# mic-rud/Learned-Compression-of-Point-Cloud-Geometry-and-Attributes

Measured on AMD Instinct MI355X. Metric: encode+decode Mpoints/sec, higher is better.
Workload: dtype f32

## Files before the change

### learned-compression-of-point-cloud-geometry-and-attributes_amd/csrc/common.h

```cpp
#pragma once
#include <hip/hip_runtime.h>
#include <stdint.h>

#include "../../include/pcc_hip.h"

namespace pcc {

void set_error(const char* fmt, ...);

#define PCC_CHECK_HIP(expr)                                                              \
    do {                                                                                 \
        hipError_t _e = (expr);                                                          \
        if (_e != hipSuccess) {                                                          \
            pcc::set_error("%s:%d: %s -> %s", __FILE__, __LINE__, #expr, hipGetErrorString(_e)); \
            return PCC_ERR_HIP;                                                          \
        }                                                                                \
    } while (0)

#define PCC_REQUIRE(cond, ...)                      \
    do {                                            \
        if (!(cond)) {                              \
            pcc::set_error(__VA_ARGS__);            \
            return PCC_ERR_ARG;                     \
        }                                           \
// ... 10 lines not shown
    return (unsigned)b;
}

constexpr uint64_t KEY_EMPTY = 0xFFFFFFFFFFFFFFFFull;
constexpr int KEY_FIELD_BITS = 18;
constexpr uint32_t KEY_FIELD_MASK = (1u << KEY_FIELD_BITS) - 1u;
constexpr int KEY_Y_SHIFT = KEY_FIELD_BITS, KEY_X_SHIFT = 2 * KEY_FIELD_BITS, KEY_B_SHIFT = 3 * KEY_FIELD_BITS;
constexpr int COORD_BIAS = 1 << (KEY_FIELD_BITS - 1);
constexpr int COORD_LIMIT = 130000;
constexpr int BATCH_LIMIT = 1022;
constexpr int64_t COUNT_ERR_RANGE = -2;

__host__ __device__ __forceinline__ bool coord_in_range(int b, int x, int y, int z) {
    return (unsigned)b <= (unsigned)BATCH_LIMIT && (unsigned)(x + COORD_LIMIT) <= 2u * COORD_LIMIT &&
           (unsigned)(y + COORD_LIMIT) <= 2u * COORD_LIMIT && (unsigned)(z + COORD_LIMIT) <= 2u * COORD_LIMIT;
}

__host__ __device__ __forceinline__ uint64_t pack_key(int b, int x, int y, int z) {
    return ((uint64_t)((uint32_t)b & 0x3FFu) << KEY_B_SHIFT) | ((uint64_t)((uint32_t)(x + COORD_BIAS) & KEY_FIELD_MASK) << KEY_X_SHIFT) |
           ((uint64_t)((uint32_t)(y + COORD_BIAS) & KEY_FIELD_MASK) << KEY_Y_SHIFT) | (uint64_t)((uint32_t)(z + COORD_BIAS) & KEY_FIELD_MASK);
}

__host__ __device__ __forceinline__ uint32_t key_z(uint64_t key) { return (uint32_t)key & KEY_FIELD_MASK; }
__host__ __device__ __forceinline__ uint32_t key_y(uint64_t key) { return (uint32_t)(key >> KEY_Y_SHIFT) & KEY_FIELD_MASK; }
__host__ __device__ __forceinline__ uint32_t key_x(uint64_t key) { return (uint32_t)(key >> KEY_X_SHIFT) & KEY_FIELD_MASK; }

__device__ __forceinline__ uint64_t hash_key(uint64_t k) {
    k ^= k >> 30; k *= 0xbf58476d1ce4e5b9ull;
    k ^= k >> 27; k *= 0x94d049bb133111ebull;
    k ^= k >> 31;
    return k;
}

__device__ __forceinline__ uint64_t table_slot0(uint64_t key, uint64_t mask, int shift) {
    const uint32_t z = key_z(key);
    const uint32_t lo = (uint32_t)(key >> (shift + 3)), hi = (uint32_t)(key >> 32);
    uint32_t h = lo * 0x9E3779B1u + hi * 0x85EBCA77u;
    h ^= h >> 15; h *= 0x2C1B3C6Du;
    h ^= h >> 12; h *= 0x297A2D39u;
    h ^= h >> 15;
    return (((uint64_t)h << 3) | (((z >> shift) + (h >> 29)) & 7u)) & mask;
}
constexpr uint64_t TABLE_PROBE_STEP = 8;

__host__ __device__ __forceinline__ int grid_shift_of(int tensor_stride) {
    int s = 0;
    if (tensor_stride > 0 && (tensor_stride & (tensor_stride - 1)) == 0)
        while ((1 << s) < tensor_stride) ++s;
    return s;
}

__device__ __forceinline__ int table_find(const uint64_t* __restrict__ keys, const int32_t* __restrict__ vals,
                                          uint64_t mask, int shift, uint64_t key) {
    const uint64_t slot0 = table_slot0(key, mask, shift);
    uint64_t slot = slot0;
    for (uint64_t probe = 0; probe <= mask; probe += TABLE_PROBE_STEP) {
        const uint64_t k = keys[slot];
        if (k == key) return vals[slot];
        if (k == KEY_EMPTY) return -1;
        slot = (slot + TABLE_PROBE_STEP) & mask;
    }
    for (uint64_t probe = 1; probe <= mask; ++probe) {
        slot = (slot0 + probe) & mask;
        const uint64_t k = keys[slot];
        if (k == key) return vals[slot];
        if (k == KEY_EMPTY) return -1;
    }
    return -1;
}

__device__ __forceinline__ uint64_t table_claim(uint64_t* keys, uint64_t mask, int shift, uint64_t key) {
    const uint64_t slot0 = table_slot0(key, mask, shift);
    uint64_t slot = slot0;
    for (uint64_t probe = 0; probe <= mask; probe += TABLE_PROBE_STEP) {
// ... 35 lines not shown
```

### learned-compression-of-point-cloud-geometry-and-attributes_amd/csrc/coords.hip

```cpp
#include <stdarg.h>
#include <stdio.h>
#include <stdlib.h>

#include "common.h"
#include "first_rows.h"
#include "sort.h"

namespace pcc {

static thread_local char g_err[512] = "";
void set_error(const char* fmt, ...) {
    va_list ap;
    va_start(ap, fmt);
    vsnprintf(g_err, sizeof(g_err), fmt, ap);
    va_end(ap);
}
const char* last_error() { return g_err; }

constexpr int SCAN_BLOCK = 256;
constexpr int SCAN_ITEMS = 4;
constexpr int SCAN_TILE = SCAN_BLOCK * SCAN_ITEMS;

__device__ __forceinline__ int wave_inclusive_scan(int v, int lane) {
#pragma unroll
// ... 271 lines not shown
    __shared__ int4 rows[64];
    __shared__ unsigned rm[64];
    __shared__ unsigned hits_s;
    const int64_t row0 = (int64_t)blockIdx.x * 64;
    if (threadIdx.x < 64) {
        const int64_t r = row0 + threadIdx.x;
        rows[threadIdx.x] = (r < n_out) ? reinterpret_cast<const int4*>(out_coords)[r] : make_int4(0, 0, 0, 0);
        rm[threadIdx.x] = 0u;
    }
    if (threadIdx.x == 0) hits_s = 0u;
    __syncthreads();
    unsigned myhits = 0u;
    const int total = 64 * K;
    for (int e = threadIdx.x; e < total; e += 256) {
        const int lr = e / K, k = e - lr * K;
        const int64_t r = row0 + lr;
        if (r >= n_out) break;
        int dx, dy, dz;
        kernel_offset(ks, k, dx, dy, dz);
        const int4 c = rows[lr];
        const int x = c.y + dx * step, y = c.z + dy * step, z = c.w + dz * step;
        int idx = -1;
        const bool on_grid = parent_pitch <= 0 || (((x % parent_pitch) | (y % parent_pitch) | (z % parent_pitch)) == 0);
        if (on_grid) idx = table_find(keys, vals, mask, shift, pack_key(c.x, x, y, z));
        nbr[r * K + k] = idx;
        if (idx >= 0) { atomicOr(&rm[lr], 1u << k); ++myhits; }
    }
    if (myhits) atomicAdd(&hits_s, myhits);
    __syncthreads();
    if (row_mask && threadIdx.x < 64 && row0 + threadIdx.x < n_out) row_mask[row0 + threadIdx.x] = rm[threadIdx.x];
    if (threadIdx.x == 0 && pair_count && !row_mask && hits_s) atomicAdd(pair_count, (unsigned long long)hits_s);
}

template <bool POW2>
__global__ __launch_bounds__(256) void kernel_map27_kernel(const int32_t* __restrict__ out_coords, int64_t n_out,
                                                           const uint64_t* __restrict__ keys,
                                                           const int32_t* __restrict__ vals, uint64_t mask, int shift,
                                                           int step, int parent_pitch, int32_t* __restrict__ nbr,
                                                           uint32_t* __restrict__ row_mask,
                                                           unsigned long long* __restrict__ pair_count) {
    __shared__ uint64_t rowkey[64];
    __shared__ uint64_t dkey[27];
    __shared__ unsigned rm[64];
    __shared__ unsigned hits_s;
    __shared__ unsigned short queue[64 * 27];
    __shared__ int queue_n;
    const int64_t row0 = (int64_t)blockIdx.x * 64;
    if (threadIdx.x < 64) {
        const int64_t r = row0 + threadIdx.x;
        const int4 c = (r < n_out) ? reinterpret_cast<const int4*>(out_coords)[r] : make_int4(0, 0, 0, 0);
        rowkey[threadIdx.x] = pack_key(c.x, c.y, c.z, c.w);
        rm[threadIdx.x] = 0u;
    }
    if (threadIdx.x == 255) queue_n = 0;
    if (threadIdx.x >= 64 && threadIdx.x < 64 + 27) {
        const int k = threadIdx.x - 64;
        const int64_t dx = (int64_t)(k % 3 - 1) * step, dy = (int64_t)((k / 3) % 3 - 1) * step, dz = (int64_t)(k / 9 - 1) * step;
        dkey[k] = (uint64_t)(dx * (1ll << KEY_X_SHIFT) + dy * (1ll << KEY_Y_SHIFT) + dz);
    }
    if (threadIdx.x == 0) hits_s = 0u;
    __syncthreads();
    const int nrows = (int)((n_out - row0 < 64) ? (n_out - row0) : 64);
    const int total = nrows * 27;
    unsigned myhits = 0u;
    auto off_grid_key = [&](uint64_t key) {
        if (POW2) {
            const uint32_t m = (uint32_t)(parent_pitch - 1);
            return ((((uint32_t)key | (uint32_t)(key >> KEY_Y_SHIFT) | (uint32_t)(key >> KEY_X_SHIFT)) & m) != 0u);
        }
        const int z = (int)key_z(key) - COORD_BIAS, y = (int)key_y(key) - COORD_BIAS, x = (int)key_x(key) - COORD_BIAS;
        return (x % parent_pitch) != 0 || (y % parent_pitch) != 0 || (z % parent_pitch) != 0;
    };
    constexpr int U = 7;
    {
        uint64_t key[U], got[U];
        uint32_t slot[U];
        int val[U];
        bool live[U];
        int lr = threadIdx.x / 27, k = threadIdx.x - lr * 27;
#pragma unroll
        for (int j = 0; j < U; ++j) {
            const int e = threadIdx.x + 256 * j;
            const bool valid = e < total;
            key[j] = rowkey[valid ? lr : 0] + dkey[k];
            live[j] = valid && (parent_pitch <= 0 || !off_grid_key(key[j]));
            slot[j] = (uint32_t)table_slot0(key[j], mask, shift);
            lr += 9;
            k += 13;
            if (k >= 27) { k -= 27; ++lr; }
        }
#pragma unroll
        for (int j = 0; j < U; ++j) {
            got[j] = live[j] ? keys[slot[j]] : KEY_EMPTY;
            val[j] = live[j] ? vals[slot[j]] : -1;
        }
        lr = threadIdx.x / 27;
        k = threadIdx.x - lr * 27;
#pragma unroll
        for (int j = 0; j < U; ++j) {
            const int e = threadIdx.x + 256 * j;
            const int lr_j = lr, k_j = k;
            lr += 9;
            k += 13;
            if (k >= 27) { k -= 27; ++lr; }
            if (e >= total) continue;
            int idx = -1;
            if (live[j] && got[j] != KEY_EMPTY) {
                if (got[j] == key[j]) idx = val[j];
                else {
                    queue[atomicAdd(&queue_n, 1)] = (unsigned short)e;
                    continue;
                }
            }
            nbr[row0 * 27 + e] = idx;
            if (idx >= 0) { atomicOr(&rm[lr_j], 1u << k_j); ++myhits; }
        }
    }
    __syncthreads();
    const int qn = queue_n;
    for (int qi = threadIdx.x; qi < qn; qi += 256) {
        const int e = queue[qi];
        const int lr = e / 27, k = e - lr * 27;
        const uint64_t key = rowkey[lr] + dkey[k];
        const uint64_t slot0 = table_slot0(key, mask, shift);
        uint64_t kk[4];
        int vv[4];
#pragma unroll
        for (int i = 0; i < 4; ++i) {
            const uint64_t sl = (slot0 + (uint64_t)(i + 1) * TABLE_PROBE_STEP) & mask;
            kk[i] = keys[sl];
            vv[i] = vals[sl];
        }
        int idx = -1;
        bool open = true;
        const int lane_slots = (int)((mask + TABLE_PROBE_STEP) / TABLE_PROBE_STEP);
#pragma unroll
        for (int i = 0; i < 4; ++i) {
            if (!open) break;
            if (i + 1 >= lane_slots) break;
            if (kk[i] == key) { idx = vv[i]; open = false; }
            else if (kk[i] == KEY_EMPTY) { idx = -1; open = false; }
        }
        if (open) idx = table_find(keys, vals, mask, shift, key);
        nbr[row0 * 27 + e] = idx;
        if (idx >= 0) { atomicOr(&rm[lr], 1u << k); ++myhits; }
    }
    if (myhits) atomicAdd(&hits_s, myhits);
    __syncthreads();
    if (row_mask && threadIdx.x < nrows) row_mask[row0 + threadIdx.x] = rm[threadIdx.x];
    if (threadIdx.x == 0 && pair_count && !row_mask && hits_s) atomicAdd(pair_count, (unsigned long long)hits_s);
}

__global__ __launch_bounds__(256) void pair_count_kernel(const uint32_t* __restrict__ row_mask, int64_t n,
                                                         unsigned long long* __restrict__ pair_count) {
    __shared__ unsigned long long ws[4];
    unsigned long long v = 0;
    for (int64_t i = (int64_t)blockIdx.x * 256 + threadIdx.x; i < n; i += (int64_t)gridDim.x * 256) v += __popc(row_mask[i]);
#pragma unroll
    for (int d = 32; d >= 1; d >>= 1) v += __shfl_xor(v, d, 64);
    if ((threadIdx.x & 63) == 0) ws[threadIdx.x >> 6] = v;
    __syncthreads();
    if (threadIdx.x == 0) {
        const unsigned long long t = ws[0] + ws[1] + ws[2] + ws[3];
        if (t) atomicAdd(pair_count, t);
    }
}

__global__ __launch_bounds__(256) void gather_rows_kernel(const float* __restrict__ src, int c,
                                                          const int32_t* __restrict__ idx, int64_t n,
                                                          float* __restrict__ out, int accumulate) {
    const int64_t total = n * c;
    for (int64_t e = (int64_t)blockIdx.x * blockDim.x + threadIdx.x; e < total; e += (int64_t)gridDim.x * blockDim.x) {
        const int64_t r = e / c;
        const int col = (int)(e - r * c);
        const int32_t s = idx[r];
        const float v = (s >= 0) ? src[(int64_t)s * c + col] : 0.0f;
        out[e] = accumulate ? out[e] + v : v;
    }
}

__global__ __launch_bounds__(256) void scatter_rows_kernel(const float* __restrict__ src, int c,
// ... 148 lines not shown
int pcc_children(const int32_t* coords, int64_t n, int32_t ts, int32_t ksize, uint64_t* keys, int32_t* vals,
                 int64_t cap, int32_t* scratch, int32_t* out_coords, int64_t* out_count, void* stream) {
    PCC_REQUIRE(ksize == 2 || ksize == 3, "pcc_children: kernel size must be 2 or 3");
    PCC_REQUIRE(ts >= 2 && (ts % 2) == 0, "pcc_children: tensor stride %d is not even", ts);
    const int K = ksize * ksize * ksize;
    GenChildren gen{coords, n, ksize, ts / 2, grid_shift_of(ts / 2)};
    return unique_coords(gen, n * K, keys, vals, cap, scratch, out_coords, out_count, as_stream(stream));
}

int32_t pcc_small_paths(int32_t mask) {
    const int before = pcc::small_paths_value();
    if (mask >= 0) pcc::g_small_paths = mask & 7;
    return before;
}

int pcc_kernel_map(const int32_t* out_coords, int64_t n_out, const uint64_t* in_keys, const int32_t* in_vals,
                   int64_t in_cap, int32_t ksize, int32_t step, int32_t sign, int32_t* nbr, uint32_t* row_mask,
                   int64_t* pair_count, void* stream) {
    PCC_REQUIRE(ksize >= 1 && ksize <= 3, "pcc_kernel_map: kernel size must be 1..3");
    PCC_REQUIRE(sign == 1 || sign == -1, "pcc_kernel_map: sign must be +1/-1");
    PCC_REQUIRE(in_cap > 0 && (in_cap & (in_cap - 1)) == 0, "pcc_kernel_map: bad capacity");
    if (pair_count) PCC_CHECK_HIP(hipMemsetAsync(pair_count, 0, sizeof(int64_t), as_stream(stream)));
    if (n_out <= 0) return PCC_OK;
    const int K = ksize * ksize * ksize;
    PCC_REQUIRE(step >= 1, "pcc_kernel_map: step must be >= 1");
    const int in_stride = sign > 0 ? step : 2 * step;
    const int pitch = sign > 0 ? 0 : 2 * step;
    const bool pow2 = pitch == 0 || (pitch & (pitch - 1)) == 0;
    unsigned long long* pc = reinterpret_cast<unsigned long long*>(pair_count);
    const uint64_t tmask = (uint64_t)(in_cap - 1);
    const int tshift = grid_shift_of(in_stride);
    const unsigned nb = blocks_for(n_out, 64);
    hipStream_t st = as_stream(stream);
    if (ksize == 3) {
        if (pow2) hipLaunchKernelGGL(kernel_map27_kernel<true>, dim3(nb), dim3(256), 0, st, out_coords, n_out, in_keys, in_vals, tmask, tshift,
                                     sign * step, pitch, nbr, row_mask, pc);
        else hipLaunchKernelGGL(kernel_map27_kernel<false>, dim3(nb), dim3(256), 0, st, out_coords, n_out, in_keys, in_vals, tmask, tshift,
                                sign * step, pitch, nbr, row_mask, pc);
    } else {
        hipLaunchKernelGGL(kernel_map_kernel, dim3(nb), dim3(256), 0, st, out_coords, n_out, in_keys, in_vals, tmask, tshift, ksize, K,
                           sign * step, pitch, nbr, row_mask, pc);
    }
    if (pair_count && row_mask)
        hipLaunchKernelGGL(pair_count_kernel, dim3(blocks_for(n_out, 256 * 16, 512)), dim3(256), 0, st, row_mask, n_out, pc);
    PCC_LAUNCH_CHECK();
    return PCC_OK;
}

int pcc_pair_count(const uint32_t* row_mask, int64_t n_out, int64_t* pair_count, void* stream) {
    PCC_REQUIRE(pair_count != nullptr, "pcc_pair_count: no output");
    hipStream_t st = as_stream(stream);
    PCC_CHECK_HIP(hipMemsetAsync(pair_count, 0, sizeof(int64_t), st));
    if (n_out <= 0) return PCC_OK;
    hipLaunchKernelGGL(pair_count_kernel, dim3(blocks_for(n_out, 256 * 16, 512)), dim3(256), 0, st, row_mask, n_out,
                       reinterpret_cast<unsigned long long*>(pair_count));
    PCC_LAUNCH_CHECK();
    return PCC_OK;
}

int pcc_gather_rows(const float* src, int32_t c, const int32_t* idx, int64_t n, float* out, int32_t accumulate,
                    void* stream) {
    if (n <= 0 || c <= 0) return PCC_OK;
    hipLaunchKernelGGL(gather_rows_kernel, dim3(blocks_for(n * c, 256, 65536)), dim3(256), 0, as_stream(stream), src, c,
                       idx, n, out, accumulate);
    PCC_LAUNCH_CHECK();
    return PCC_OK;
}

int pcc_scatter_rows(const float* src, int32_t c, const int32_t* idx, int64_t n, float* out, void* stream) {
    if (n <= 0 || c <= 0) return PCC_OK;
    hipLaunchKernelGGL(scatter_rows_kernel, dim3(blocks_for(n * c, 256, 65536)), dim3(256), 0, as_stream(stream), src,
// ... 50 lines not shown
```

### learned-compression-of-point-cloud-geometry-and-attributes_amd/csrc/select.hip

```cpp
#include <stdlib.h>

#include "common.h"
#include "sort_small.h"

namespace pcc {

constexpr int TK_STRIDE = 264;
constexpr int TK_LDS_BATCHES = 16;

__device__ __forceinline__ uint32_t float_key(float v) {
    if (v != v) return 0xFFFFFFFFu;
    if (v == 0.0f) v = 0.0f;
    const uint32_t u = __float_as_uint(v);
    return (u & 0x80000000u) ? ~u : (u | 0x80000000u);
}

struct Key96 { uint32_t w[3]; };

__device__ __forceinline__ Key96 make_key(float logit, int4 c) {
    const uint64_t lo = ~pack_key(c.x, c.y, c.z, c.w);
    Key96 k;
    k.w[0] = float_key(logit);
    k.w[1] = (uint32_t)(lo >> 32);
    k.w[2] = (uint32_t)lo;
// ... 224 lines not shown
        return true;
    });
    const int nb = st[2];
    for (int i = t; i < n; i += 1024) {
        const int4 c = reinterpret_cast<const int4*>(coords)[i];
        uint8_t m = 0;
        if (c.x == 0 && nb <= 12) m = cmp_prefix(make_key(logits[(int64_t)i * ld], c), st, nb) >= 0 ? 1 : 0;
        mask[i] = m;
    }
    for (int i = t; i < TK_STRIDE; i += 1024) state[i] = i < 8 ? st[i] : 0;
}

__global__ __launch_bounds__(256) void mask_bit_counts_kernel(const uint32_t* __restrict__ row_mask, int64_t n,
                                                              uint32_t* __restrict__ counts) {
    __shared__ unsigned c[27];
    if (threadIdx.x < 27) c[threadIdx.x] = 0u;
    __syncthreads();
    unsigned mine[27];
#pragma unroll
    for (int b = 0; b < 27; ++b) mine[b] = 0u;
    for (int64_t i0 = (int64_t)blockIdx.x * 256; i0 < n; i0 += (int64_t)gridDim.x * 256) {
        const int64_t i = i0 + threadIdx.x;
        const uint32_t m = (i < n) ? row_mask[i] : 0u;
#pragma unroll
        for (int b = 0; b < 27; ++b) mine[b] += (unsigned)__popcll(__ballot((m >> b) & 1u));
    }
    if ((threadIdx.x & 63) == 0) {
#pragma unroll
        for (int b = 0; b < 27; ++b)
            if (mine[b]) atomicAdd(&c[b], mine[b]);
    }
    __syncthreads();
    if (threadIdx.x < 27 && c[threadIdx.x]) atomicAdd(&counts[threadIdx.x], c[threadIdx.x]);
}

__device__ __forceinline__ void order_bit_positions(const uint32_t* __restrict__ counts, int* pos_s) {
    if (threadIdx.x < 27) {
        const uint32_t mine = counts[threadIdx.x];
        int rank = 0;
        for (int b = 0; b < 27; ++b) {
            const uint32_t o = counts[b];
            rank += (o < mine || (o == mine && b < (int)threadIdx.x)) ? 1 : 0;
        }
        pos_s[threadIdx.x] = 26 - rank;
    }
    __syncthreads();
}

__device__ __forceinline__ uint32_t order_key_of(uint32_t m, const int* pos_s) {
    uint32_t key = 0u;
#pragma unroll
    for (int b = 0; b < 27; ++b) key |= ((m >> b) & 1u) << pos_s[b];
    return 0x7FFFFFFu - key;
}

__global__ __launch_bounds__(256) void order_keys32_kernel(const uint32_t* __restrict__ row_mask, int64_t n,
                                                           const uint32_t* __restrict__ counts, uint32_t* __restrict__ keys) {
    __shared__ int pos_s[27];
    order_bit_positions(counts, pos_s);
    const int64_t i = (int64_t)blockIdx.x * 256 + threadIdx.x;
    if (i >= n) return;
    const uint32_t m = row_mask[i] & 0x7FFFFFFu;
    keys[i] = order_key_of(m, pos_s);
}

__global__ __launch_bounds__(256) void order_keys64_kernel(const uint32_t* __restrict__ row_mask,
                                                           const int32_t* __restrict__ coords, int64_t n,
                                                           int block_log2, int ts, const uint32_t* __restrict__ counts,
                                                           uint64_t* __restrict__ keys) {
    __shared__ int pos_s[27];
    order_bit_positions(counts, pos_s);
    const int64_t i = (int64_t)blockIdx.x * 256 + threadIdx.x;
    if (i >= n) return;
    uint64_t key = order_key_of(row_mask[i] & 0x7FFFFFFu, pos_s);
    const int4 c = reinterpret_cast<const int4*>(coords)[i];
    const uint64_t bx = (uint64_t)(((c.y / ts) + 512) >> block_log2) & 0x3FF;
    const uint64_t by = (uint64_t)(((c.z / ts) + 512) >> block_log2) & 0x3FF;
    const uint64_t bz = (uint64_t)(((c.w / ts) + 512) >> block_log2) & 0x3FF;
    key |= ((((uint64_t)(c.x & 0x3) << 30) | (bx << 20) | (by << 10) | bz) << 32);
    keys[i] = key;
}

__device__ __forceinline__ uint32_t tile_or_mask(uint32_t m) {
#pragma unroll
    for (int d = 1; d < 32; d <<= 1) m |= __shfl_xor(m, d, 64);
    return m;
// ... 203 lines not shown
    return PCC_OK;
}

int64_t pcc_order_scratch_bytes(int64_t n) { return pcc_sort_scratch_bytes(n); }

int pcc_order_rows_by_mask(const uint32_t* row_mask, const int32_t* coords, int64_t n, int32_t block_log2,
                           int32_t tensor_stride, int32_t* order, uint32_t* group_mask32, void* scratch, int64_t scratch_bytes,
                           void* stream) {
    if (n <= 0) return PCC_OK;
    PCC_REQUIRE(n < (1ll << 31), "pcc_order_rows_by_mask: too many rows");
    PCC_REQUIRE(block_log2 < 0 || coords != nullptr, "pcc_order_rows_by_mask: block ordering needs coordinates");
    PCC_REQUIRE(block_log2 <= 10, "pcc_order_rows_by_mask: block_log2 out of range");
    PCC_REQUIRE(tensor_stride >= 1, "pcc_order_rows_by_mask: bad tensor stride");
    PCC_REQUIRE(scratch_bytes >= pcc_sort_scratch_bytes(n), "pcc_order_rows_by_mask: scratch too small");
    hipStream_t st = as_stream(stream);
    const SortScratch s = carve_sort_scratch(scratch, n);
    if (small_path_enabled(0) && block_log2 < 0 && n <= RS_SMALL_N) {
        rs_small_dispatch(rs_small_rounds((int)n), [&](auto r) {
            hipLaunchKernelGGL(order_small_kernel<decltype(r)::value>, dim3(1), dim3(RS_SMALL_THREADS), 0, st, row_mask, (int)n,
                               static_cast<uint32_t*>(s.keys_a), static_cast<uint32_t*>(s.keys_b), s.vals_x, order);
        });
    } else {
        uint32_t* bit_counts = s.tail;
        PCC_CHECK_HIP(hipMemsetAsync(bit_counts, 0, 27 * sizeof(uint32_t), st));
        hipLaunchKernelGGL(mask_bit_counts_kernel, dim3(blocks_for(n, 256 * 16, 512)), dim3(256), 0, st, row_mask, n, bit_counts);
        const int begin = 0, end = block_log2 >= 0 ? 64 : 27;
        const int digit_bits = block_log2 >= 0 ? 8 : radix_sort_order_digit_bits(n);
        const bool in_b = radix_sort_result_in_b(begin, end, digit_bits);
        int32_t* va = in_b ? s.vals_x : order;
        int32_t* vb = in_b ? order : s.vals_x;
        int rc;
        if (block_log2 < 0) {
            uint32_t* ka = static_cast<uint32_t*>(s.keys_a);
            hipLaunchKernelGGL(order_keys32_kernel, dim3(blocks_for(n, 256)), dim3(256), 0, st, row_mask, n, bit_counts, ka);
            rc = radix_sort_pairs_u32(ka, static_cast<uint32_t*>(s.keys_b), va, vb, true, n, begin, end, s.counters, st, digit_bits);
        } else {
            uint64_t* ka = static_cast<uint64_t*>(s.keys_a);
            hipLaunchKernelGGL(order_keys64_kernel, dim3(blocks_for(n, 256)), dim3(256), 0, st, row_mask, coords, n, block_log2, tensor_stride,
                               bit_counts, ka);
            rc = radix_sort_pairs_u64(ka, static_cast<uint64_t*>(s.keys_b), va, vb, true, n, begin, end, s.counters, st);
        }
        if (rc) return rc;
    }
    hipLaunchKernelGGL(group_masks_kernel, dim3(blocks_for(n, 256)), dim3(256), 0, st, order, row_mask, n, group_mask32);
    PCC_LAUNCH_CHECK();
    return PCC_OK;
}

int64_t pcc_small_map_max(void) {
    static int off = -1;
    if (off < 0) { const char* e = getenv("PCC_SMALL_MAP"); off = (e && e[0] == '0') ? 1 : 0; }
    return off ? 0 : SMALL_MAP_MAX;
}

int pcc_small_kernel_map(const int32_t* out_coords, int64_t n_out, const uint64_t* in_keys, const int32_t* in_vals, int64_t in_cap,
                         int32_t ksize, int32_t step, int32_t sign, int32_t* nbr, uint32_t* row_mask, int32_t* order,
                         uint32_t* group_mask32, void* scratch, int64_t scratch_bytes, void* stream) {
    PCC_REQUIRE(ksize == 2 || ksize == 3, "pcc_small_kernel_map: kernel size must be 2 or 3");
    PCC_REQUIRE(sign == 1 || sign == -1, "pcc_small_kernel_map: sign must be +1/-1");
    PCC_REQUIRE(in_cap > 0 && (in_cap & (in_cap - 1)) == 0, "pcc_small_kernel_map: bad capacity");
    PCC_REQUIRE(step >= 1, "pcc_small_kernel_map: step must be >= 1");
    PCC_REQUIRE(n_out >= 0 && n_out <= SMALL_MAP_MAX, "pcc_small_kernel_map: %lld rows exceed %d", (long long)n_out, SMALL_MAP_MAX);
    PCC_REQUIRE(scratch_bytes >= pcc_sort_scratch_bytes(n_out), "pcc_small_kernel_map: scratch too small");
    if (n_out <= 0) return PCC_OK;
    const int in_stride = sign > 0 ? step : 2 * step;
    const int pitch = sign > 0 ? 0 : 2 * step;
    const SortScratch s = carve_sort_scratch(scratch, n_out);
    auto launch = [&](auto kernel) {
// ... 35 lines not shown
```

### learned-compression-of-point-cloud-geometry-and-attributes_amd/csrc/sort.h

```cpp
#pragma once
#include "common.h"

namespace pcc {

static inline int64_t align256(int64_t v) { return (v + 255) / 256 * 256; }

int64_t scan_block_sums_elems(int64_t m);
int scan_flags(const int32_t* flags, int64_t m, int32_t* pos, int32_t* block_sums, int64_t* total, int inclusive,
               hipStream_t st, const int32_t* err = nullptr);

int radix_sort_passes(int begin_bit, int end_bit, int digit_bits = 8);
static inline bool radix_sort_result_in_b(int begin_bit, int end_bit, int digit_bits = 8) { return radix_sort_passes(begin_bit, end_bit, digit_bits) & 1; }
int64_t radix_sort_counter_bytes(int64_t n);
int radix_sort_order_digit_bits(int64_t n);
int radix_sort_pairs_u32(uint32_t* keys_a, uint32_t* keys_b, int32_t* vals_a, int32_t* vals_b, bool vals_are_iota, int64_t n,
                         int begin_bit, int end_bit, void* counters, hipStream_t st, int digit_bits = 8);
int radix_sort_pairs_u64(uint64_t* keys_a, uint64_t* keys_b, int32_t* vals_a, int32_t* vals_b, bool vals_are_iota, int64_t n,
                         int begin_bit, int end_bit, void* counters, hipStream_t st);

}
```

### learned-compression-of-point-cloud-geometry-and-attributes_amd/csrc/sort.hip

```cpp
#include "sort_small.h"

namespace pcc {

constexpr int RS_MID_ITEMS = 8;
constexpr int RS_MID_MAX_UNITS = 64;
constexpr int RS_BIG_ITEMS = 16;

template <class K, int ROUNDS, int DB>
__global__ __launch_bounds__(RS_SMALL_THREADS) void radix_sort_small_kernel(K* ka, K* kb, int32_t* va, int32_t* vb, int iota, int n,
                                                                           int begin_bit, int end_bit, int passes) {
    radix_sort_small_body<K, ROUNDS, DB>(ka, kb, va, vb, iota, n, begin_bit, end_bit, passes);
}

template <class K, int ITEMS, int DB>
__global__ __launch_bounds__(256) void radix_count_kernel(const K* __restrict__ keys, int64_t n, int shift, unsigned dmask,
                                                          int64_t nunits, int32_t* __restrict__ counts) {
    constexpr int ND = 1 << DB;
    __shared__ int cnt[ND];
#pragma unroll
    for (int d = threadIdx.x; d < ND; d += 256) cnt[d] = 0;
    __syncthreads();
    const int64_t base = (int64_t)blockIdx.x * (256 * ITEMS);
    K key[ITEMS];
#pragma unroll
    for (int j = 0; j < ITEMS; ++j) {
        const int64_t i = base + (int64_t)j * 256 + threadIdx.x;
        key[j] = (i < n) ? keys[i] : (K)0;
    }
#pragma unroll
    for (int j = 0; j < ITEMS; ++j)
        if (base + (int64_t)j * 256 + threadIdx.x < n) atomicAdd(&cnt[(unsigned)(key[j] >> shift) & dmask], 1);
    __syncthreads();
#pragma unroll
    for (int d = threadIdx.x; d < ND; d += 256) counts[(int64_t)d * nunits + blockIdx.x] = cnt[d];
}

__global__ __launch_bounds__(256) void radix_rowscan_kernel(int32_t* __restrict__ counts, int64_t nunits, int32_t* __restrict__ totals) {
    __shared__ int wsum[4];
    __shared__ int carry_s;
    const int t = threadIdx.x, lane = t & 63, w = t >> 6;
    int32_t* row = counts + (int64_t)blockIdx.x * nunits;
    if (t == 0) carry_s = 0;
    __syncthreads();
    for (int64_t base = 0; base < nunits; base += 1024) {
        const int64_t i = base + 4 * (int64_t)t;
        int f[4];
        int v = 0;
#pragma unroll
        for (int j = 0; j < 4; ++j) {
            f[j] = (i + j < nunits) ? row[i + j] : 0;
            v += f[j];
        }
        const int inc = wave_inclusive_scan_i32(v, lane);
        if (lane == 63) wsum[w] = inc;
        __syncthreads();
        int pre = carry_s;
        for (int ww = 0; ww < w; ++ww) pre += wsum[ww];
        int ex = pre + inc - v;
#pragma unroll
        for (int j = 0; j < 4; ++j) {
            if (i + j < nunits) row[i + j] = ex;
            ex += f[j];
        }
        __syncthreads();
        if (t == 255) carry_s = pre + inc;
        __syncthreads();
    }
    if (t == 0) totals[blockIdx.x] = carry_s;
}

template <class K, int ITEMS, bool SELF_PREFIX, int DB>
__global__ __launch_bounds__(256) void radix_scatter_kernel(const K* __restrict__ src, K* __restrict__ dst, const int32_t* __restrict__ vs,
                                                            int32_t* __restrict__ vd, int iota, int64_t n, int shift, unsigned dmask,
                                                            int64_t nunits, const int32_t* __restrict__ counts,
                                                            const int32_t* __restrict__ totals) {
    constexpr int WAVE_KEYS = 64 * ITEMS, WG_KEYS = 4 * WAVE_KEYS;
    constexpr int ND = 1 << DB, DH = ND / 256;
    __shared__ K skey[WG_KEYS];
    __shared__ int32_t sval[WG_KEYS];
    __shared__ int cnt[4][ND];
    __shared__ int lbase[ND];
    __shared__ int gbase[ND];
    __shared__ int wsum[4], wsum2[4];
    const int t = threadIdx.x, lane = t & 63, w = t >> 6;
    const uint64_t lt = (1ull << lane) - 1ull;
    for (int i = t; i < 4 * ND; i += 256) (&cnt[0][0])[i] = 0;
    const int64_t base0 = (int64_t)blockIdx.x * WG_KEYS;
    const int64_t wbase = base0 + (int64_t)w * WAVE_KEYS;
    K key[ITEMS];
    int32_t val[ITEMS];
#pragma unroll
    for (int j = 0; j < ITEMS; ++j) {
        const int64_t i = wbase + j * 64 + lane;
        key[j] = (i < n) ? src[i] : (K)0;
        val[j] = (i < n) ? (iota ? (int32_t)i : vs[i]) : 0;
    }
    int pre[DH], total[DH];
#pragma unroll
    for (int h = 0; h < DH; ++h) {
        const int d = h * 256 + t;
        if (SELF_PREFIX) {
            const int32_t* row = counts + (int64_t)d * nunits;
            pre[h] = 0;
            total[h] = 0;
            for (int64_t u = 0; u < nunits; ++u) {
                const int c = row[u];
                total[h] += c;
                pre[h] += (u < (int64_t)blockIdx.x) ? c : 0;
            }
        } else {
            pre[h] = counts[(int64_t)d * nunits + blockIdx.x];
            total[h] = totals[d];
        }
    }
    __syncthreads();
#pragma unroll
    for (int j = 0; j < ITEMS; ++j)
        if (wbase + j * 64 + lane < n) atomicAdd(&cnt[w][(unsigned)(key[j] >> shift) & dmask], 1);
    __syncthreads();
    int gcarry = 0, lcarry = 0;
#pragma unroll
    for (int h = 0; h < DH; ++h) {
        const int d = h * 256 + t;
        const int c0 = cnt[0][d], c1 = cnt[1][d], c2 = cnt[2][d], c3 = cnt[3][d];
        const int mine = c0 + c1 + c2 + c3;
        const int inc = wave_inclusive_scan_i32(total[h], lane);
        const int linc = wave_inclusive_scan_i32(mine, lane);
// ... 25 lines not shown
        }
        __builtin_amdgcn_wave_barrier();
        if (active && below == 0) cnt[w][d] = base + __popcll(same);
        __builtin_amdgcn_wave_barrier();
    }
    __syncthreads();
    const int nk = (int)((n - base0 < WG_KEYS) ? (n - base0) : WG_KEYS);
    for (int i = t; i < nk; i += 256) {
        const K k = skey[i];
        const unsigned d = (unsigned)(k >> shift) & dmask;
        const int64_t pos = (int64_t)gbase[d] + (i - lbase[d]);
        dst[pos] = k;
        vd[pos] = sval[i];
    }
}

int radix_sort_passes(int begin_bit, int end_bit, int digit_bits) {
    return end_bit > begin_bit ? (end_bit - begin_bit + digit_bits - 1) / digit_bits : 0;
}

int radix_sort_order_digit_bits(int64_t n) {
    const int64_t mid_units = (n + 256 * RS_MID_ITEMS - 1) / (256 * RS_MID_ITEMS);
    return (n > RS_SMALL_N && mid_units <= RS_MID_MAX_UNITS) ? 8 : 9;
}

int64_t radix_sort_counter_bytes(int64_t n) {
    const int64_t mid = (n + 256 * RS_MID_ITEMS - 1) / (256 * RS_MID_ITEMS), big = (n + 256 * RS_BIG_ITEMS - 1) / (256 * RS_BIG_ITEMS);
    const int64_t nunits = mid <= RS_MID_MAX_UNITS ? mid : big;
    return align256(512 * (nunits > 0 ? nunits : 1) * 4) + 2048;
}

template <class K, int DB>
static int radix_sort_pairs(K* ka, K* kb, int32_t* va, int32_t* vb, bool iota, int64_t n, int begin_bit, int end_bit, void* counters,
                            hipStream_t st) {
    constexpr int ND = 1 << DB;
    const int passes = radix_sort_passes(begin_bit, end_bit, DB);
    PCC_REQUIRE(passes >= 1 && end_bit <= (int)(8 * sizeof(K)) && begin_bit >= 0, "radix sort: bad bit range [%d, %d)", begin_bit, end_bit);
    PCC_REQUIRE(n < (1ll << 31), "radix sort: too many keys (%lld)", (long long)n);
    if (n <= 0) return PCC_OK;
    if (n <= RS_SMALL_N) {
        rs_small_dispatch(rs_small_rounds((int)n), [&](auto r) {
            hipLaunchKernelGGL((radix_sort_small_kernel<K, decltype(r)::value, DB>), dim3(1), dim3(RS_SMALL_THREADS), 0, st, ka, kb, va, vb,
                               iota ? 1 : 0, (int)n, begin_bit, end_bit, passes);
        });
        PCC_LAUNCH_CHECK();
        return PCC_OK;
    }
    const int64_t mid_units = (n + 256 * RS_MID_ITEMS - 1) / (256 * RS_MID_ITEMS);
    const bool mid = mid_units <= RS_MID_MAX_UNITS;
    const int64_t nunits = mid ? mid_units : (n + 256 * RS_BIG_ITEMS - 1) / (256 * RS_BIG_ITEMS);
    int32_t* counts = reinterpret_cast<int32_t*>(counters);
    int32_t* totals = counts + align256((int64_t)ND * nunits * 4) / 4;
    K* src = ka;
    K* dst = kb;
    int32_t* vs = va;
    int32_t* vd = vb;
    for (int p = 0; p < passes; ++p) {
        const int shift = begin_bit + DB * p;
        const unsigned dmask = (end_bit - shift >= DB) ? (unsigned)(ND - 1) : ((1u << (end_bit - shift)) - 1u);
        const int io = (iota && p == 0) ? 1 : 0;
        if (mid) {
            hipLaunchKernelGGL((radix_count_kernel<K, RS_MID_ITEMS, DB>), dim3((unsigned)nunits), dim3(256), 0, st, src, n, shift, dmask, nunits, counts);
            hipLaunchKernelGGL((radix_scatter_kernel<K, RS_MID_ITEMS, true, DB>), dim3((unsigned)nunits), dim3(256), 0, st, src, dst, vs, vd, io, n,
                               shift, dmask, nunits, counts, totals);
        } else {
            hipLaunchKernelGGL((radix_count_kernel<K, RS_BIG_ITEMS, DB>), dim3((unsigned)nunits), dim3(256), 0, st, src, n, shift, dmask, nunits, counts);
            hipLaunchKernelGGL(radix_rowscan_kernel, dim3(ND), dim3(256), 0, st, counts, nunits, totals);
            hipLaunchKernelGGL((radix_scatter_kernel<K, RS_BIG_ITEMS, false, DB>), dim3((unsigned)nunits), dim3(256), 0, st, src, dst, vs, vd, io, n,
                               shift, dmask, nunits, counts, totals);
        }
        K* tk = src; src = dst; dst = tk;
        int32_t* tv = vs; vs = vd; vd = tv;
    }
    PCC_LAUNCH_CHECK();
    return PCC_OK;
}

int radix_sort_pairs_u32(uint32_t* keys_a, uint32_t* keys_b, int32_t* vals_a, int32_t* vals_b, bool vals_are_iota, int64_t n, int begin_bit,
                         int end_bit, void* counters, hipStream_t st, int digit_bits) {
    if (digit_bits == 9) return radix_sort_pairs<uint32_t, 9>(keys_a, keys_b, vals_a, vals_b, vals_are_iota, n, begin_bit, end_bit, counters, st);
    return radix_sort_pairs<uint32_t, 8>(keys_a, keys_b, vals_a, vals_b, vals_are_iota, n, begin_bit, end_bit, counters, st);
}

int radix_sort_pairs_u64(uint64_t* keys_a, uint64_t* keys_b, int32_t* vals_a, int32_t* vals_b, bool vals_are_iota, int64_t n, int begin_bit,
                         int end_bit, void* counters, hipStream_t st) {
    return radix_sort_pairs<uint64_t, 8>(keys_a, keys_b, vals_a, vals_b, vals_are_iota, n, begin_bit, end_bit, counters, st);
}

}
```

Baseline: 8.949.

## Share hashes across z-neighbours in map27 and fuse order-key build into radix sort

The 27-neighbour map kernel now has each thread handle three z-adjacent offsets. It reuses the run hash when those keys fall in the same hash run, reorders rows so run-crossing rows are grouped, and stages results in shared memory for vectorised int4 stores. The block size drops to 192 threads. Separately, for large sorts, the order-key generation kernel is fused into the first radix pass: keys are computed from the row masks through a per-block 3x512 lookup table instead of being written to memory first. This removes one kernel and one key round trip, but adds LUT setup to every count and scatter block.

```diff
diff --git a/learned-compression-of-point-cloud-geometry-and-attributes_amd/csrc/common.h b/learned-compression-of-point-cloud-geometry-and-attributes_amd/csrc/common.h
--- a/learned-compression-of-point-cloud-geometry-and-attributes_amd/csrc/common.h
+++ b/learned-compression-of-point-cloud-geometry-and-attributes_amd/csrc/common.h
@@ -66,14 +66,23 @@
     return k;
 }
 
-__device__ __forceinline__ uint64_t table_slot0(uint64_t key, uint64_t mask, int shift) {
-    const uint32_t z = key_z(key);
-    const uint32_t lo = (uint32_t)(key >> (shift + 3)), hi = (uint32_t)(key >> 32);
+__device__ __forceinline__ uint32_t table_run_lo(uint64_t key, int shift) { return (uint32_t)(key >> (shift + 3)); }
+__device__ __forceinline__ uint32_t table_run_hi(uint64_t key) { return (uint32_t)(key >> 32); }
+
+__device__ __forceinline__ uint32_t table_run_hash(uint32_t lo, uint32_t hi) {
     uint32_t h = lo * 0x9E3779B1u + hi * 0x85EBCA77u;
     h ^= h >> 15; h *= 0x2C1B3C6Du;
     h ^= h >> 12; h *= 0x297A2D39u;
     h ^= h >> 15;
+    return h;
+}
+
+__device__ __forceinline__ uint64_t table_run_slot(uint32_t h, uint32_t z, uint64_t mask, int shift) {
     return (((uint64_t)h << 3) | (((z >> shift) + (h >> 29)) & 7u)) & mask;
+}
+
+__device__ __forceinline__ uint64_t table_slot0(uint64_t key, uint64_t mask, int shift) {
+    return table_run_slot(table_run_hash(table_run_lo(key, shift), table_run_hi(key)), key_z(key), mask, shift);
 }
 constexpr uint64_t TABLE_PROBE_STEP = 8;
 
diff --git a/learned-compression-of-point-cloud-geometry-and-attributes_amd/csrc/coords.hip b/learned-compression-of-point-cloud-geometry-and-attributes_amd/csrc/coords.hip
--- a/learned-compression-of-point-cloud-geometry-and-attributes_amd/csrc/coords.hip
+++ b/learned-compression-of-point-cloud-geometry-and-attributes_amd/csrc/coords.hip
@@ -327,8 +327,9 @@
     if (threadIdx.x == 0 && pair_count && !row_mask && hits_s) atomicAdd(pair_count, (unsigned long long)hits_s);
 }
 
+constexpr int MAP27_ROWS = 64, MAP27_THREADS = 192, MAP27_COLS = 3;
 template <bool POW2>
-__global__ __launch_bounds__(256) void kernel_map27_kernel(const int32_t* __restrict__ out_coords, int64_t n_out,
+__global__ __launch_bounds__(MAP27_THREADS) void kernel_map27_kernel(const int32_t* __restrict__ out_coords, int64_t n_out,
                                                            const uint64_t* __restrict__ keys,
                                                            const int32_t* __restrict__ vals, uint64_t mask, int shift,
                                                            int step, int parent_pitch, int32_t* __restrict__ nbr,
@@ -340,14 +341,25 @@
     __shared__ unsigned hits_s;
     __shared__ unsigned short queue[64 * 27];
     __shared__ int queue_n;
+    __shared__ __attribute__((aligned(16))) int32_t stage[MAP27_ROWS * 27];
+    static_assert(MAP27_ROWS == 64 && MAP27_ROWS * 9 == MAP27_THREADS * MAP27_COLS && MAP27_THREADS >= 64 + 27, "lane mapping");
+    __shared__ unsigned char rowat[64];
     const int64_t row0 = (int64_t)blockIdx.x * 64;
+    const int nrows = (int)((n_out - row0 < 64) ? (n_out - row0) : 64);
     if (threadIdx.x < 64) {
         const int64_t r = row0 + threadIdx.x;
-        const int4 c = (r < n_out) ? reinterpret_cast<const int4*>(out_coords)[r] : make_int4(0, 0, 0, 0);
-        rowkey[threadIdx.x] = pack_key(c.x, c.y, c.z, c.w);
+        const bool valid = r < n_out;
+        const int4 c = valid ? reinterpret_cast<const int4*>(out_coords)[r] : make_int4(0, 0, 0, 0);
+        const uint64_t key = pack_key(c.x, c.y, c.z, c.w), dzkey = (uint64_t)(int64_t)step;
+        rowkey[threadIdx.x] = key;
         rm[threadIdx.x] = 0u;
-    }
-    if (threadIdx.x == 255) queue_n = 0;
+        const uint32_t lo = table_run_lo(key, shift);
+        const bool crosses = valid && (table_run_lo(key - dzkey, shift) != lo || table_run_lo(key + dzkey, shift) != lo);
+        const uint64_t cb = __ballot(crosses), sb = __ballot(valid && !crosses), below = (1ull << threadIdx.x) - 1ull;
+        const int at = !valid ? (int)threadIdx.x : crosses ? __popcll(cb & below) : __popcll(cb) + __popcll(sb & below);
+        rowat[at] = (unsigned char)threadIdx.x;
+    }
+    if (threadIdx.x == MAP27_THREADS - 1) queue_n = 0;
     if (threadIdx.x >= 64 && threadIdx.x < 64 + 27) {
         const int k = threadIdx.x - 64;
         const int64_t dx = (int64_t)(k % 3 - 1) * step, dy = (int64_t)((k / 3) % 3 - 1) * step, dz = (int64_t)(k / 9 - 1) * step;
@@ -355,7 +367,6 @@
     }
     if (threadIdx.x == 0) hits_s = 0u;
     __syncthreads();
-    const int nrows = (int)((n_out - row0 < 64) ? (n_out - row0) : 64);
     const int total = nrows * 27;
     unsigned myhits = 0u;
     auto off_grid_key = [&](uint64_t key) {
@@ -366,54 +377,78 @@
         const int z = (int)key_z(key) - COORD_BIAS, y = (int)key_y(key) - COORD_BIAS, x = (int)key_x(key) - COORD_BIAS;
         return (x % parent_pitch) != 0 || (y % parent_pitch) != 0 || (z % parent_pitch) != 0;
     };
-    constexpr int U = 7;
     {
-        uint64_t key[U], got[U];
-        uint32_t slot[U];
-        int val[U];
-        bool live[U];
-        int lr = threadIdx.x / 27, k = threadIdx.x - lr * 27;
+        constexpr int U = MAP27_COLS;
+        uint64_t key[U][3], got[U][3];
+        uint32_t slot[U][3];
+        int val[U][3];
+        bool live[U][3];
+        const uint64_t dzkey = (uint64_t)(int64_t)step;
+        const int ncols = nrows * 9;
+        int p = threadIdx.x / 9, c9 = threadIdx.x - p * 9;
+        int lr[U];
 #pragma unroll
         for (int j = 0; j < U; ++j) {
-            const int e = threadIdx.x + 256 * j;
-            const bool valid = e < total;
-            key[j] = rowkey[valid ? lr : 0] + dkey[k];
-            live[j] = valid && (parent_pitch <= 0 || !off_grid_key(key[j]));
-            slot[j] = (uint32_t)table_slot0(key[j], mask, shift);
-            lr += 9;
-            k += 13;
-            if (k >= 27) { k -= 27; ++lr; }
+            const bool valid = threadIdx.x + MAP27_THREADS * j < ncols;
+            lr[j] = valid ? rowat[p] : 0;
+            const uint64_t centre = rowkey[lr[j]] + dkey[9 + c9];
+            key[j][0] = centre - dzkey;
+            key[j][1] = centre;
+            key[j][2] = centre + dzkey;
+            uint32_t lo[3];
+#pragma unroll
+            for (int d = 0; d < 3; ++d) {
+                live[j][d] = valid && (parent_pitch <= 0 || !off_grid_key(key[j][d]));
+                lo[d] = table_run_lo(key[j][d], shift);
+            }
+            const uint32_t hi = table_run_hi(centre);
+            const uint32_t first = live[j][1] ? lo[1] : (live[j][0] ? lo[0] : lo[2]);
+#pragma unroll
+            for (int d = 0; d < 3; ++d) lo[d] = live[j][d] ? lo[d] : first;
+            const bool other0 = lo[0] != lo[1], other2 = lo[2] != lo[1];
+            const uint32_t h_a = table_run_hash(lo[1], hi);
+            uint32_t h_b = h_a;
+            if (other0 || other2) h_b = table_run_hash(other0 ? lo[0] : lo[2], hi);
+            uint32_t h_c = h_b;
+            if (other0 && other2 && lo[2] != lo[0]) h_c = table_run_hash(lo[2], hi);
+            const uint32_t h[3] = {other0 ? h_b : h_a, h_a, other2 ? (other0 ? h_c : h_b) : h_a};
+#pragma unroll
+            for (int d = 0; d < 3; ++d) slot[j][d] = (uint32_t)table_run_slot(h[d], key_z(key[j][d]), mask, shift);
+            p += 21;
+            c9 += 3;
+            if (c9 >= 9) { c9 -= 9; ++p; }
         }
 #pragma unroll
         for (int j = 0; j < U; ++j) {
-            got[j] = live[j] ? keys[slot[j]] : KEY_EMPTY;
-            val[j] = live[j] ? vals[slot[j]] : -1;
-        }
-        lr = threadIdx.x / 27;
-        k = threadIdx.x - lr * 27;
+#pragma unroll
+            for (int d = 0; d < 3; ++d) {
+                got[j][d] = live[j][d] ? keys[slot[j][d]] : KEY_EMPTY;
+                val[j][d] = live[j][d] ? vals[slot[j][d]] : -1;
+            }
+        }
+        c9 = threadIdx.x % 9;
 #pragma unroll
         for (int j = 0; j < U; ++j) {
-            const int e = threadIdx.x + 256 * j;
-            const int lr_j = lr, k_j = k;
-            lr += 9;
-            k += 13;
-            if (k >= 27) { k -= 27; ++lr; }
-            if (e >= total) continue;
-            int idx = -1;
-            if (live[j] && got[j] != KEY_EMPTY) {
-                if (got[j] == key[j]) idx = val[j];
-                else {
-                    queue[atomicAdd(&queue_n, 1)] = (unsigned short)e;
-                    continue;
-                }
+            const int lr_j = lr[j], c_j = c9;
+            c9 += 3;
+            if (c9 >= 9) c9 -= 9;
+            if (threadIdx.x + MAP27_THREADS * j >= ncols) continue;
+            unsigned bits = 0u;
+#pragma unroll
+            for (int d = 0; d < 3; ++d) {
+                const int k = c_j + 9 * d, e = 27 * lr_j + k;
+                const int idx = got[j][d] == key[j][d] ? val[j][d] : -1;
+                stage[e] = idx;
+                bits |= (idx >= 0 ? 1u : 0u) << k;
+                if (got[j][d] != key[j][d] && got[j][d] != KEY_EMPTY) queue[atomicAdd(&queue_n, 1)] = (unsigned short)e;
             }
-            nbr[row0 * 27 + e] = idx;
-            if (idx >= 0) { atomicOr(&rm[lr_j], 1u << k_j); ++myhits; }
+            myhits += __popc(bits);
+            if (bits) atomicOr(&rm[lr_j], bits);
         }
     }
     __syncthreads();
     const int qn = queue_n;
-    for (int qi = threadIdx.x; qi < qn; qi += 256) {
+    for (int qi = threadIdx.x; qi < qn; qi += MAP27_THREADS) {
         const int e = queue[qi];
         const int lr = e / 27, k = e - lr * 27;
         const uint64_t key = rowkey[lr] + dkey[k];
@@ -437,11 +472,15 @@
             else if (kk[i] == KEY_EMPTY) { idx = -1; open = false; }
         }
         if (open) idx = table_find(keys, vals, mask, shift, key);
-        nbr[row0 * 27 + e] = idx;
+        stage[e] = idx;
         if (idx >= 0) { atomicOr(&rm[lr], 1u << k); ++myhits; }
     }
     if (myhits) atomicAdd(&hits_s, myhits);
     __syncthreads();
+    int32_t* out = nbr + row0 * 27;
+    const int nvec = ((reinterpret_cast<uintptr_t>(out) & 15u) == 0u) ? total >> 2 : 0;
+    for (int i = threadIdx.x; i < nvec; i += MAP27_THREADS) reinterpret_cast<int4*>(out)[i] = reinterpret_cast<const int4*>(stage)[i];
+    for (int i = 4 * nvec + threadIdx.x; i < total; i += MAP27_THREADS) out[i] = stage[i];
     if (row_mask && threadIdx.x < nrows) row_mask[row0 + threadIdx.x] = rm[threadIdx.x];
     if (threadIdx.x == 0 && pair_count && !row_mask && hits_s) atomicAdd(pair_count, (unsigned long long)hits_s);
 }
@@ -656,11 +695,12 @@
     const int tshift = grid_shift_of(in_stride);
     const unsigned nb = blocks_for(n_out, 64);
     hipStream_t st = as_stream(stream);
+    static_assert(MAP27_ROWS == 64, "nb counts 64 rows per workgroup for every map kernel");
     if (ksize == 3) {
-        if (pow2) hipLaunchKernelGGL(kernel_map27_kernel<true>, dim3(nb), dim3(256), 0, st, out_coords, n_out, in_keys, in_vals, tmask, tshift,
-                                     sign * step, pitch, nbr, row_mask, pc);
-        else hipLaunchKernelGGL(kernel_map27_kernel<false>, dim3(nb), dim3(256), 0, st, out_coords, n_out, in_keys, in_vals, tmask, tshift,
-                                sign * step, pitch, nbr, row_mask, pc);
+        if (pow2) hipLaunchKernelGGL(kernel_map27_kernel<true>, dim3(nb), dim3(MAP27_THREADS), 0, st, out_coords, n_out, in_keys, in_vals, tmask,
+                                     tshift, sign * step, pitch, nbr, row_mask, pc);
+        else hipLaunchKernelGGL(kernel_map27_kernel<false>, dim3(nb), dim3(MAP27_THREADS), 0, st, out_coords, n_out, in_keys, in_vals, tmask,
+                                tshift, sign * step, pitch, nbr, row_mask, pc);
     } else {
         hipLaunchKernelGGL(kernel_map_kernel, dim3(nb), dim3(256), 0, st, out_coords, n_out, in_keys, in_vals, tmask, tshift, ksize, K,
                            sign * step, pitch, nbr, row_mask, pc);
diff --git a/learned-compression-of-point-cloud-geometry-and-attributes_amd/csrc/select.hip b/learned-compression-of-point-cloud-geometry-and-attributes_amd/csrc/select.hip
--- a/learned-compression-of-point-cloud-geometry-and-attributes_amd/csrc/select.hip
+++ b/learned-compression-of-point-cloud-geometry-and-attributes_amd/csrc/select.hip
@@ -280,26 +280,6 @@
     }
     __syncthreads();
     if (threadIdx.x < 27 && c[threadIdx.x]) atomicAdd(&counts[threadIdx.x], c[threadIdx.x]);
-}
-
-__device__ __forceinline__ void order_bit_positions(const uint32_t* __restrict__ counts, int* pos_s) {
-    if (threadIdx.x < 27) {
-        const uint32_t mine = counts[threadIdx.x];
-        int rank = 0;
-        for (int b = 0; b < 27; ++b) {
-            const uint32_t o = counts[b];
-            rank += (o < mine || (o == mine && b < (int)threadIdx.x)) ? 1 : 0;
-        }
-        pos_s[threadIdx.x] = 26 - rank;
-    }
-    __syncthreads();
-}
-
-__device__ __forceinline__ uint32_t order_key_of(uint32_t m, const int* pos_s) {
-    uint32_t key = 0u;
-#pragma unroll
-    for (int b = 0; b < 27; ++b) key |= ((m >> b) & 1u) << pos_s[b];
-    return 0x7FFFFFFu - key;
 }
 
 __global__ __launch_bounds__(256) void order_keys32_kernel(const uint32_t* __restrict__ row_mask, int64_t n,
@@ -569,8 +549,12 @@
         int rc;
         if (block_log2 < 0) {
             uint32_t* ka = static_cast<uint32_t*>(s.keys_a);
-            hipLaunchKernelGGL(order_keys32_kernel, dim3(blocks_for(n, 256)), dim3(256), 0, st, row_mask, n, bit_counts, ka);
-            rc = radix_sort_pairs_u32(ka, static_cast<uint32_t*>(s.keys_b), va, vb, true, n, begin, end, s.counters, st, digit_bits);
+            if (n > RS_SMALL_N) {
+                rc = radix_sort_order_u32(row_mask, bit_counts, ka, static_cast<uint32_t*>(s.keys_b), va, vb, n, s.counters, st, digit_bits);
+            } else {
+                hipLaunchKernelGGL(order_keys32_kernel, dim3(blocks_for(n, 256)), dim3(256), 0, st, row_mask, n, bit_counts, ka);
+                rc = radix_sort_pairs_u32(ka, static_cast<uint32_t*>(s.keys_b), va, vb, true, n, begin, end, s.counters, st, digit_bits);
+            }
         } else {
             uint64_t* ka = static_cast<uint64_t*>(s.keys_a);
             hipLaunchKernelGGL(order_keys64_kernel, dim3(blocks_for(n, 256)), dim3(256), 0, st, row_mask, coords, n, block_log2, tensor_stride,
diff --git a/learned-compression-of-point-cloud-geometry-and-attributes_amd/csrc/sort.h b/learned-compression-of-point-cloud-geometry-and-attributes_amd/csrc/sort.h
--- a/learned-compression-of-point-cloud-geometry-and-attributes_amd/csrc/sort.h
+++ b/learned-compression-of-point-cloud-geometry-and-attributes_amd/csrc/sort.h
@@ -18,4 +18,45 @@
 int radix_sort_pairs_u64(uint64_t* keys_a, uint64_t* keys_b, int32_t* vals_a, int32_t* vals_b, bool vals_are_iota, int64_t n,
                          int begin_bit, int end_bit, void* counters, hipStream_t st);
 
+__device__ __forceinline__ void order_bit_positions(const uint32_t* __restrict__ counts, int* pos_s) {
+    if (threadIdx.x < 27) {
+        const uint32_t mine = counts[threadIdx.x];
+        int rank = 0;
+        for (int b = 0; b < 27; ++b) {
+            const uint32_t o = counts[b];
+            rank += (o < mine || (o == mine && b < (int)threadIdx.x)) ? 1 : 0;
+        }
+        pos_s[threadIdx.x] = 26 - rank;
+    }
+    __syncthreads();
 }
+
+__device__ __forceinline__ uint32_t order_key_of(uint32_t m, const int* pos_s) {
+    uint32_t key = 0u;
+#pragma unroll
+    for (int b = 0; b < 27; ++b) key |= ((m >> b) & 1u) << pos_s[b];
+    return 0x7FFFFFFu - key;
+}
+
+constexpr int ORDER_LUT_SIZE = 3 * 512;
+__device__ __forceinline__ void order_key_tables(const uint32_t* __restrict__ counts, int* pos_s, uint32_t* lut) {
+    order_bit_positions(counts, pos_s);
+    for (int i = threadIdx.x; i < ORDER_LUT_SIZE; i += blockDim.x) {
+        const int third = i >> 9;
+        const uint32_t v = (uint32_t)i & 511u;
+        uint32_t image = 0u;
+#pragma unroll
+        for (int b = 0; b < 9; ++b) image |= ((v >> b) & 1u) << pos_s[9 * third + b];
+        lut[i] = image;
+    }
+    __syncthreads();
+}
+
+__device__ __forceinline__ uint32_t order_key_from_tables(uint32_t m, const uint32_t* lut) {
+    return 0x7FFFFFFu - (lut[m & 511u] | lut[512 + ((m >> 9) & 511u)] | lut[1024 + ((m >> 18) & 511u)]);
+}
+
+int radix_sort_order_u32(const uint32_t* row_mask, const uint32_t* mask_counts, uint32_t* keys_a, uint32_t* keys_b, int32_t* vals_a,
+                         int32_t* vals_b, int64_t n, void* counters, hipStream_t st, int digit_bits);
+
+}
diff --git a/learned-compression-of-point-cloud-geometry-and-attributes_amd/csrc/sort.hip b/learned-compression-of-point-cloud-geometry-and-attributes_amd/csrc/sort.hip
--- a/learned-compression-of-point-cloud-geometry-and-attributes_amd/csrc/sort.hip
+++ b/learned-compression-of-point-cloud-geometry-and-attributes_amd/csrc/sort.hip
@@ -12,11 +12,21 @@
     radix_sort_small_body<K, ROUNDS, DB>(ka, kb, va, vb, iota, n, begin_bit, end_bit, passes);
 }
 
-template <class K, int ITEMS, int DB>
+template <class K, bool FROM_MASKS>
+__device__ __forceinline__ K radix_load_key(const K* __restrict__ src, int64_t i, const uint32_t* key_lut) {
+    if constexpr (FROM_MASKS) return (K)order_key_from_tables((uint32_t)src[i] & 0x7FFFFFFu, key_lut);
+    else return src[i];
+}
+
+template <class K, int ITEMS, int DB, bool FROM_MASKS = false>
 __global__ __launch_bounds__(256) void radix_count_kernel(const K* __restrict__ keys, int64_t n, int shift, unsigned dmask,
-                                                          int64_t nunits, int32_t* __restrict__ counts) {
+                                                          int64_t nunits, int32_t* __restrict__ counts,
+                                                          const uint32_t* __restrict__ mask_counts) {
     constexpr int ND = 1 << DB;
     __shared__ int cnt[ND];
+    __shared__ int pos_s[27];
+    __shared__ uint32_t key_lut[FROM_MASKS ? ORDER_LUT_SIZE : 1];
+    if (FROM_MASKS) order_key_tables(mask_counts, pos_s, key_lut);
 #pragma unroll
     for (int d = threadIdx.x; d < ND; d += 256) cnt[d] = 0;
     __syncthreads();
@@ -25,7 +35,7 @@
 #pragma unroll
     for (int j = 0; j < ITEMS; ++j) {
         const int64_t i = base + (int64_t)j * 256 + threadIdx.x;
-        key[j] = (i < n) ? keys[i] : (K)0;
+        key[j] = (i < n) ? radix_load_key<K, FROM_MASKS>(keys, i, key_lut) : (K)0;
     }
 #pragma unroll
     for (int j = 0; j < ITEMS; ++j)
@@ -69,11 +79,11 @@
     if (t == 0) totals[blockIdx.x] = carry_s;
 }
 
-template <class K, int ITEMS, bool SELF_PREFIX, int DB>
+template <class K, int ITEMS, bool SELF_PREFIX, int DB, bool FROM_MASKS = false>
 __global__ __launch_bounds__(256) void radix_scatter_kernel(const K* __restrict__ src, K* __restrict__ dst, const int32_t* __restrict__ vs,
                                                             int32_t* __restrict__ vd, int iota, int64_t n, int shift, unsigned dmask,
                                                             int64_t nunits, const int32_t* __restrict__ counts,
-                                                            const int32_t* __restrict__ totals) {
+                                                            const int32_t* __restrict__ totals, const uint32_t* __restrict__ mask_counts) {
     constexpr int WAVE_KEYS = 64 * ITEMS, WG_KEYS = 4 * WAVE_KEYS;
     constexpr int ND = 1 << DB, DH = ND / 256;
     __shared__ K skey[WG_KEYS];
@@ -82,8 +92,11 @@
     __shared__ int lbase[ND];
     __shared__ int gbase[ND];
     __shared__ int wsum[4], wsum2[4];
+    __shared__ int pos_s[27];
     const int t = threadIdx.x, lane = t & 63, w = t >> 6;
     const uint64_t lt = (1ull << lane) - 1ull;
+    __shared__ uint32_t key_lut[FROM_MASKS ? ORDER_LUT_SIZE : 1];
+    if (FROM_MASKS) order_key_tables(mask_counts, pos_s, key_lut);
     for (int i = t; i < 4 * ND; i += 256) (&cnt[0][0])[i] = 0;
     const int64_t base0 = (int64_t)blockIdx.x * WG_KEYS;
     const int64_t wbase = base0 + (int64_t)w * WAVE_KEYS;
@@ -92,7 +105,7 @@
 #pragma unroll
     for (int j = 0; j < ITEMS; ++j) {
         const int64_t i = wbase + j * 64 + lane;
-        key[j] = (i < n) ? src[i] : (K)0;
+        key[j] = (i < n) ? radix_load_key<K, FROM_MASKS>(src, i, key_lut) : (K)0;
         val[j] = (i < n) ? (iota ? (int32_t)i : vs[i]) : 0;
     }
     int pre[DH], total[DH];
@@ -184,12 +197,14 @@
 
 template <class K, int DB>
 static int radix_sort_pairs(K* ka, K* kb, int32_t* va, int32_t* vb, bool iota, int64_t n, int begin_bit, int end_bit, void* counters,
-                            hipStream_t st) {
+                            hipStream_t st, const uint32_t* row_mask = nullptr, const uint32_t* mask_counts = nullptr) {
     constexpr int ND = 1 << DB;
     const int passes = radix_sort_passes(begin_bit, end_bit, DB);
     PCC_REQUIRE(passes >= 1 && end_bit <= (int)(8 * sizeof(K)) && begin_bit >= 0, "radix sort: bad bit range [%d, %d)", begin_bit, end_bit);
     PCC_REQUIRE(n < (1ll << 31), "radix sort: too many keys (%lld)", (long long)n);
     if (n <= 0) return PCC_OK;
+    PCC_REQUIRE(!row_mask || (std::is_same<K, uint32_t>::value && n > RS_SMALL_N && begin_bit == 0 && mask_counts),
+                "radix sort: keys from masks need 32-bit keys and more than %d rows", RS_SMALL_N);
     if (n <= RS_SMALL_N) {
         rs_small_dispatch(rs_small_rounds((int)n), [&](auto r) {
             hipLaunchKernelGGL((radix_sort_small_kernel<K, decltype(r)::value, DB>), dim3(1), dim3(RS_SMALL_THREADS), 0, st, ka, kb, va, vb,
@@ -211,15 +226,28 @@
         const int shift = begin_bit + DB * p;
         const unsigned dmask = (end_bit - shift >= DB) ? (unsigned)(ND - 1) : ((1u << (end_bit - shift)) - 1u);
         const int io = (iota && p == 0) ? 1 : 0;
-        if (mid) {
-            hipLaunchKernelGGL((radix_count_kernel<K, RS_MID_ITEMS, DB>), dim3((unsigned)nunits), dim3(256), 0, st, src, n, shift, dmask, nunits, counts);
-            hipLaunchKernelGGL((radix_scatter_kernel<K, RS_MID_ITEMS, true, DB>), dim3((unsigned)nunits), dim3(256), 0, st, src, dst, vs, vd, io, n,
-                               shift, dmask, nunits, counts, totals);
-        } else {
-            hipLaunchKernelGGL((radix_count_kernel<K, RS_BIG_ITEMS, DB>), dim3((unsigned)nunits), dim3(256), 0, st, src, n, shift, dmask, nunits, counts);
-            hipLaunchKernelGGL(radix_rowscan_kernel, dim3(ND), dim3(256), 0, st, counts, nunits, totals);
-            hipLaunchKernelGGL((radix_scatter_kernel<K, RS_BIG_ITEMS, false, DB>), dim3((unsigned)nunits), dim3(256), 0, st, src, dst, vs, vd, io, n,
-                               shift, dmask, nunits, counts, totals);
+        auto launch = [&](auto items, auto self_prefix, auto from_masks, const K* in) {
+            constexpr int ITEMS = decltype(items)::value;
+            constexpr bool SELF = decltype(self_prefix)::value, MASKS = decltype(from_masks)::value;
+            hipLaunchKernelGGL((radix_count_kernel<K, ITEMS, DB, MASKS>), dim3((unsigned)nunits), dim3(256), 0, st, in, n, shift, dmask, nunits, counts,
+                               mask_counts);
+            if (!SELF) hipLaunchKernelGGL(radix_rowscan_kernel, dim3(ND), dim3(256), 0, st, counts, nunits, totals);
+            hipLaunchKernelGGL((radix_scatter_kernel<K, ITEMS, SELF, DB, MASKS>), dim3((unsigned)nunits), dim3(256), 0, st, in, dst, vs, vd, io, n,
+                               shift, dmask, nunits, counts, totals, mask_counts);
+        };
+        const std::integral_constant<int, RS_MID_ITEMS> mid_items;
+        const std::integral_constant<int, RS_BIG_ITEMS> big_items;
+        bool from_masks = false;
+        if constexpr (std::is_same<K, uint32_t>::value) {
+            if (p == 0 && row_mask) {
+                from_masks = true;
+                if (mid) launch(mid_items, std::true_type(), std::true_type(), row_mask);
+                else launch(big_items, std::false_type(), std::true_type(), row_mask);
+            }
+        }
+        if (!from_masks) {
+            if (mid) launch(mid_items, std::true_type(), std::false_type(), src);
+            else launch(big_items, std::false_type(), std::false_type(), src);
         }
         K* tk = src; src = dst; dst = tk;
         int32_t* tv = vs; vs = vd; vd = tv;
@@ -234,6 +262,12 @@
     return radix_sort_pairs<uint32_t, 8>(keys_a, keys_b, vals_a, vals_b, vals_are_iota, n, begin_bit, end_bit, counters, st);
 }
 
+int radix_sort_order_u32(const uint32_t* row_mask, const uint32_t* mask_counts, uint32_t* keys_a, uint32_t* keys_b, int32_t* vals_a,
+                         int32_t* vals_b, int64_t n, void* counters, hipStream_t st, int digit_bits) {
+    if (digit_bits == 9) return radix_sort_pairs<uint32_t, 9>(keys_a, keys_b, vals_a, vals_b, true, n, 0, 27, counters, st, row_mask, mask_counts);
+    return radix_sort_pairs<uint32_t, 8>(keys_a, keys_b, vals_a, vals_b, true, n, 0, 27, counters, st, row_mask, mask_counts);
+}
+
 int radix_sort_pairs_u64(uint64_t* keys_a, uint64_t* keys_b, int32_t* vals_a, int32_t* vals_b, bool vals_are_iota, int64_t n, int begin_bit,
                          int end_bit, void* counters, hipStream_t st) {
     return radix_sort_pairs<uint64_t, 8>(keys_a, keys_b, vals_a, vals_b, vals_are_iota, n, begin_bit, end_bit, counters, st);
```

New measurement: 8.975, median of 6. About the same (+0.3%).
